# ziyu0425/PDE-Solver

Hardware: NVIDIA B200
Metric: GDOF/s (higher is better)
Workload: dtype f64

## Files before the change

### include/pde_b200.h

```cpp
#ifndef PDE_B200_H
#define PDE_B200_H

#include <stdint.h>

#ifdef __cplusplus
extern "C" {
#endif

typedef struct pde_ctx pde_ctx;

const char* pde_last_error(void);
int pde_version(void);
int pde_device_count(int32_t* count);
int pde_ctx_create(int device, pde_ctx** out);
int pde_ctx_destroy(pde_ctx* ctx);
int64_t pde_ctx_launch_count(pde_ctx* ctx);
int pde_ctx_sync(pde_ctx* ctx);
int pde_timer_start(pde_ctx* ctx);
int pde_timer_stop(pde_ctx* ctx, double* elapsed_ms);

int pde_host_alloc(uint64_t bytes, void** out);
int pde_host_free(void* p);

int pde_nccl_unique_id(const char* libnccl_path, void* id128 );
// ... 72 lines not shown
  pde_bc bc;
} pde_heat_params;

int pde_heat_solve(pde_ctx* ctx, const pde_heat_params* p, const pde_solver_opts* o,
                   const double* u0, double* values_out, double* times_out, pde_stats* st);

typedef struct pde_heat_state pde_heat_state;
int pde_heat_open(pde_ctx* ctx, const pde_heat_params* p, const pde_solver_opts* o,
                  pde_heat_state** out);
int pde_heat_set_state(pde_heat_state* s, const double* u_host );
int pde_heat_step(pde_heat_state* s, int nsteps, pde_stats* st);
int pde_heat_get_state(pde_heat_state* s, double* u_host );
int pde_heat_advance_batch(pde_heat_state* s, int nreq, const double* const* u_in_host,
                           double* const* u_out_host, pde_stats* st);
int64_t pde_heat_local_nverts(pde_heat_state* s);
int pde_heat_close(pde_heat_state* s);

typedef struct pde_wheat_params {
  int32_t dim;
  int32_t n[3];
  double lo[3], hi[3];
  int32_t weight_rpow;
  int32_t weight_sin_axis1;
  int32_t weight_degree;
  int32_t steady;
  double diffusivity;
  double dt;
  int32_t num_steps;
  int32_t snapshot_stride;
  double source_value;
  double T_initial;
  pde_bc bc;
  int32_t weight_kind;
  int32_t has_core;
  double core_radius;
  double core_diffusivity;
  int32_t initial_type;
  int32_t reserved0;
  double initial_amplitude;
  double initial_wavenumber;
} pde_wheat_params;
int pde_wheat_solve(pde_ctx* ctx, const pde_wheat_params* p, const pde_solver_opts* o,
                    double* values_out , double* times_out, pde_stats* st);
typedef struct pde_wheat_state pde_wheat_state;
int pde_wheat_open(pde_ctx* ctx, const pde_wheat_params* p, const pde_solver_opts* o, pde_wheat_state** out);
int pde_wheat_set_state(pde_wheat_state* s, const double* u_host );
int pde_wheat_step(pde_wheat_state* s, int nsteps, pde_stats* st);
int pde_wheat_get_state(pde_wheat_state* s, double* u_host );
int64_t pde_wheat_local_nverts(pde_wheat_state* s);
int pde_wheat_close(pde_wheat_state* s);
int pde_wheat_level_coefs(pde_ctx* ctx, const pde_wheat_params* p, int level, int32_t n_out[3], double* coef_out);

typedef struct pde_elast_params {
  int32_t dim;
  int32_t n[3];
  double L[3];
  double E;
  double nu;
  double body[3];
  int32_t quantity;
  int32_t plane_stress;
  double area;
} pde_elast_params;

int pde_elasticity_solve(pde_ctx* ctx, const pde_elast_params* p, const pde_solver_opts* o,
                         double* field_out, double* disp_out, pde_stats* st, pde_stats* st_proj);

enum { PDE_OP_HEAT = 0, PDE_OP_MASS = 1, PDE_OP_STIFFNESS = 2, PDE_OP_ELASTICITY = 3 };

typedef struct pde_op_params {
  int32_t kind;
  int32_t dim;
  int32_t n[3];
  double L[3];
  double alpha;
  double beta;
  double lam, mu;
  pde_bc bc;
  int32_t variant;
} pde_op_params;

int pde_op_table(const pde_op_params* p, double* table, int32_t* ncomp);
int pde_op_apply(pde_ctx* ctx, const pde_op_params* p, const double* x, double* y);
int pde_op_bench(pde_ctx* ctx, const pde_op_params* p, int reps, int warmup, double* ms_per_apply,
                 int64_t* ndofs);
int pde_op_sweep(pde_ctx* ctx, const pde_op_params* p, int32_t mode, double c1, double c2, const double* x,
                 const double* b, const double* xprev, double* y, double* dots);
int pde_op_bench_mode(pde_ctx* ctx, const pde_op_params* p, int32_t mode, int32_t reps, int32_t warmup,
                      double* ms_per_launch, int64_t* ndofs);
int pde_op_solve(pde_ctx* ctx, const pde_op_params* p, const pde_solver_opts* o, const double* b,
                 double* x, pde_stats* st);

int pde_op_manufactured(pde_ctx* ctx, const pde_op_params* p, const pde_solver_opts* o, double* rel_l2_error,
                        pde_stats* st);

#ifdef __cplusplus
}
#endif
#endif
```

### pde_solver_b200/_lib.py

```python
import ctypes as C
import os
import threading

import numpy as np

_HERE = os.path.dirname(os.path.abspath(__file__))
LIB_PATH = os.environ.get("PDE_B200_LIB") or os.path.join(_HERE, "libpde_b200.so")


class PdeError(RuntimeError):
    pass


class Bc(C.Structure):
    _fields_ = [("face_on", C.c_int32 * 6), ("face_val", C.c_double * 6), ("side_excludes_xends", C.c_int32)]


class SolverOpts(C.Structure):
    _fields_ = [("rtol", C.c_double), ("max_iters", C.c_int32), ("precond", C.c_int32),
                ("cheby_degree", C.c_int32), ("check_every", C.c_int32), ("cheby_ratio", C.c_double),
                ("verify_residual", C.c_int32), ("reserved", C.c_int32 * 3)]


class Stats(C.Structure):
# ... 148 lines not shown
        return ms.value

    def close(self):
        if self.handle:
            lib().pde_ctx_destroy(self.handle)
            self.handle = C.c_void_p()


_ctx = None


def default_context():
    global _ctx
    if _ctx is None:
        _ctx = Context()
    return _ctx


def device_count():
    n = C.c_int32(0)
    check(lib().pde_device_count(C.byref(n)))
    return int(n.value)


def nccl_library_path():
    try:
        import nvidia.nccl as _n
        base = list(_n.__path__)[0]
        p = os.path.join(base, "lib", "libnccl.so.2")
        if os.path.exists(p):
            return p
    except Exception:
        pass
    return None


def nccl_unique_id(libnccl_path=None):
    buf = (C.c_char * 128)()
    path = libnccl_path.encode() if libnccl_path else None
    check(lib().pde_nccl_unique_id(path, buf))
    return bytes(buf)


def mesh_counts(dim, n):
    nv, nc = C.c_int64(), C.c_int64()
    check(lib().pde_mesh_counts(int(dim), i3(n), C.byref(nv), C.byref(nc)))
    return nv.value, nc.value


def slab_partition(dim, n, rank, world, level=0):
    z0, nzl, nzg = C.c_int32(), C.c_int32(), C.c_int32()
    check(lib().pde_slab_partition(int(dim), i3(n), int(rank), int(world), int(level), C.byref(z0), C.byref(nzl),
                                   C.byref(nzg)))
    return z0.value, nzl.value, nzg.value


def op_params(kind, dim, n, L, alpha=1.0, beta=1.0, lam=0.0, mu=0.0, bc=None, variant=0):
    p = OpParams()
    p.kind = OP[kind] if isinstance(kind, str) else int(kind)
    p.dim = int(dim)
    p.n = i3(n)
    p.L = d3(L)
    p.alpha, p.beta, p.lam, p.mu = float(alpha), float(beta), float(lam), float(mu)
    p.bc = bc if bc is not None else Bc()
    p.variant = int(variant)
    return p


def op_table(p):
    nc = C.c_int32()
    check(lib().pde_op_table(C.byref(p), None, C.byref(nc)))
    t = np.zeros((27, 15, nc.value, nc.value))
    check(lib().pde_op_table(C.byref(p), ptr(t), C.byref(nc)))
    return t


def op_apply(ctx, p, x):
    x = np.ascontiguousarray(x, dtype=np.float64)
    y = np.empty_like(x)
    check(lib().pde_op_apply(ctx.handle, C.byref(p), ptr(x), ptr(y)))
    return y


def op_sweep(ctx, p, mode, x, b=None, xprev=None, c1=0.0, c2=0.0):
    x = np.ascontiguousarray(x, dtype=np.float64)
    b = None if b is None else np.ascontiguousarray(b, dtype=np.float64)
    xprev = None if xprev is None else np.ascontiguousarray(xprev, dtype=np.float64)
    y = np.empty_like(x)
    dots = np.zeros(2)
    check(lib().pde_op_sweep(ctx.handle, C.byref(p), int(mode), C.c_double(c1), C.c_double(c2), ptr(x),
                             ptr(b) if b is not None else None, ptr(xprev) if xprev is not None else None, ptr(y),
                             ptr(dots)))
    return y, dots


def op_bench_mode(ctx, p, mode, reps=20, warmup=3):
    ms, nd = C.c_double(), C.c_int64()
    check(lib().pde_op_bench_mode(ctx.handle, C.byref(p), int(mode), int(reps), int(warmup), C.byref(ms), C.byref(nd)))
    return ms.value, nd.value


def op_solve(ctx, p, b, opts=None):
    b = np.ascontiguousarray(b, dtype=np.float64)
    x = np.empty_like(b)
    st = Stats()
    o = opts if opts is not None else make_opts()
    check(lib().pde_op_solve(ctx.handle, C.byref(p), C.byref(o), ptr(b), ptr(x), C.byref(st)))
    return x, st.as_dict()


def comm_info(ctx):
    hp, ne, na = C.c_int32(), C.c_int64(), C.c_int64()
    check(lib().pde_comm_info(ctx.handle, C.byref(hp), C.byref(ne), C.byref(na)))
    return {"halo_path": {0: "none", 1: "nccl send/recv", 2: "peer-memory mailbox kernel (cudaIpc over NVLink)"}[hp.value],
            "halo_exchanges": ne.value, "allreduces": na.value}


def halo_check(ctx, dim, n, ncomp=1, depth=1, reps=4):
    bad = C.c_int64(0)
    check(lib().pde_halo_check(ctx.handle, int(dim), i3(n), int(ncomp), int(depth), int(reps), C.byref(bad)))
    return int(bad.value)


def halo_bench(ctx, dim, n, ncomp=1, reps=50):
    ms, nb = C.c_double(), C.c_int64()
    check(lib().pde_halo_bench(ctx.handle, int(dim), i3(n), int(ncomp), int(reps), C.byref(ms), C.byref(nb)))
    return ms.value, nb.value


def op_manufactured(ctx, p, opts=None):
    err = C.c_double()
    st = Stats()
    o = opts if opts is not None else make_opts()
    check(lib().pde_op_manufactured(ctx.handle, C.byref(p), C.byref(o), C.byref(err), C.byref(st)))
    return err.value, st.as_dict()


def op_bench(ctx, p, reps=20, warmup=3):
    ms, nd = C.c_double(), C.c_int64()
    check(lib().pde_op_bench(ctx.handle, C.byref(p), int(reps), int(warmup), C.byref(ms), C.byref(nd)))
    return ms.value, nd.value


class PinnedArray:

    def __init__(self, n):
        self.ptr = C.c_void_p()
        check(lib().pde_host_alloc(C.c_uint64(int(n) * 8), C.byref(self.ptr)))
        self.array = np.ctypeslib.as_array(C.cast(self.ptr, C.POINTER(C.c_double)), shape=(int(n),))

    def free(self):
        if self.ptr:
            self.array = None
            lib().pde_host_free(self.ptr)
            self.ptr = C.c_void_p()


class HeatStepper:

    def __init__(self, ctx, dim, n, L, diffusivity, dt, T_initial=0.0, bc=None, source_value=0.0, steady=False,
                 opts=None):
        p = HeatParams()
        p.dim = int(dim)
        p.n = i3(n)
        p.L = d3(L)
        p.diffusivity = float(diffusivity)
# ... 41 lines not shown
```

### pde_solver_b200/csrc/cabi.cu

```cuda
#include <cmath>
#include <cstdlib>
#include <cstring>
#include <new>

#include "solver.cuh"

int comm_destroy(pde_ctx* c);

extern "C" int pde_ctx_create(int device, pde_ctx** out) {
  if (!out) PDE_FAIL("null out pointer");
  int ndev = 0;
  cudaError_t e = cudaGetDeviceCount(&ndev);
  if (e != cudaSuccess || ndev == 0)
    PDE_FAIL(std::string("no CUDA device available (this library has no CPU fallback): ") + cudaGetErrorString(e));
  if (device < 0 || device >= ndev) PDE_FAIL("device index out of range");
  CUDA_OK(cudaSetDevice(device));
  pde_ctx* c = new (std::nothrow) pde_ctx();
  if (!c) PDE_FAIL("out of host memory");
  c->device = device;
  cudaDeviceGetAttribute(&c->sm_count, cudaDevAttrMultiProcessorCount, device);
  CUDA_OK(cudaStreamCreateWithFlags(&c->stream, cudaStreamNonBlocking));
  CUDA_OK(cudaEventCreate(&c->ev0));
  CUDA_OK(cudaEventCreate(&c->ev1));
  CUDA_OK(cudaEventCreateWithFlags(&c->ev_poll, cudaEventDisableTiming));
// ... 551 lines not shown
    if ((rc = pipe_init(s, false))) break;
    s->pipe.nout = 0;
    if ((rc = pipe_push_snapshot(s, values_out))) break;
    times_out[snap++] = 0.0;
    const int stride = p->snapshot_stride > 0 ? p->snapshot_stride : 1;
    const int verify = s->o.verify_residual;
    for (int step = 0; step < p->num_steps; ++step) {
      pde_stats st;
      s->o.verify_residual = step == p->num_steps - 1 ? verify : -1;
      if ((rc = pde_heat_step(s, 1, &st))) break;
      acc.true_relres = st.true_relres;
      acc.iters_total += st.iters_total;
      acc.solves += st.solves;
      acc.converged &= st.converged;
      acc.levels = st.levels;
      acc.final_relres = st.final_relres;
      acc.solve_ms += st.solve_ms;
      acc.launches += st.launches;
      if ((step + 1) % stride == 0) {
        if ((rc = pipe_push_snapshot(s, values_out + snap * s->nloc))) break;
        times_out[snap++] = (step + 1) * p->dt;
      }
    }
    if (!rc) rc = pipe_drain(s);
    acc.setup_ms = s->setup_ms;
  } while (0);
  pde_heat_close(s);
  if (st_out) *st_out = acc;
  return rc;
}

static int setup_op(pde_ctx* c, const pde_op_params* p, Operator* A, int* ncomp) {
  Grid g;
  PDE_OK(make_grid(p->dim, p->n, p->L, c->rank, c->world, &g));
  BcDev bc;
  PDE_OK(make_bc(p->dim, p->n, &p->bc, &bc));
  if (p->kind == PDE_OP_ELASTICITY) {
    if (p->dim < 2) PDE_FAIL("elasticity operator needs dim 2 or 3");
    PDE_OK(A->setup_elasticity(c, g, bc, p->lam, p->mu));
  } else {
    double a = p->kind == PDE_OP_MASS ? 1.0 : (p->kind == PDE_OP_STIFFNESS ? 0.0 : p->alpha);
    double b = p->kind == PDE_OP_MASS ? 0.0 : (p->kind == PDE_OP_STIFFNESS ? 1.0 : p->beta);
    PDE_OK(A->setup_scalar(c, g, bc, a, b));
  }
  *ncomp = A->tab.ncomp;
  return 0;
}

struct OpGuard {
  Operator A;
  Field x, y, r;
  PcgWork w;
  Hierarchy mg;
  ~OpGuard() { A.release(); x.release(); y.release(); r.release(); w.release(); mg.release(); }
};

extern "C" int pde_device_count(int32_t* count) {
  int n = 0;
  if (cudaGetDeviceCount(&n) != cudaSuccess) { cudaGetLastError(); n = 0; }
  if (count) *count = n;
  return 0;
}

extern "C" int pde_op_apply(pde_ctx* c, const pde_op_params* p, const double* x, double* y) {
  if (!c || !p || !x || !y) PDE_FAIL("null argument");
  CUDA_OK(cudaSetDevice(c->device));
  OpGuard G;
  int nc;
  PDE_OK(setup_op(c, p, &G.A, &nc));
  const Grid& g = G.A.g;
  PDE_OK(G.x.alloc(c, g, nc));
  PDE_OK(G.y.alloc(c, g, nc));
  const long long nloc = (long long)g.nn[0] * g.nn[1] * g.nzl;
  DevMem dense;
  PDE_OK(dense.alloc(sizeof(double) * nloc * nc));
  PDE_OK(h2d(c, dense.p, x, sizeof(double) * nloc * nc));
  PDE_OK(launch_unpack(c, g, nc, (const double*)dense.p, G.x.p, 0));
  StencilArgs a;
  a.x = G.x.p; a.y = G.y.p; a.variant = p->variant; a.reduce_slot_xy = S_XY;
  if (c->world > 1) PDE_OK(comm_halo_exchange(c, g, nc, G.x.p));
  PDE_OK(launch_stencil(c, g, G.A.bc, G.A.dev, a));
  PDE_OK(launch_pack(c, g, nc, G.y.p, (double*)dense.p, 0));
  return d2h(c, y, dense.p, sizeof(double) * nloc * nc);
}

extern "C" int pde_op_bench(pde_ctx* c, const pde_op_params* p, int reps, int warmup, double* ms_per_apply,
                            int64_t* ndofs) {
  if (!c || !p) PDE_FAIL("null argument");
  CUDA_OK(cudaSetDevice(c->device));
  OpGuard G;
  int nc;
  PDE_OK(setup_op(c, p, &G.A, &nc));
  const Grid& g = G.A.g;
  PDE_OK(G.x.alloc(c, g, nc));
  PDE_OK(G.y.alloc(c, g, nc));
  PDE_OK(launch_fill_pattern(c, g, G.A.bc, nc, G.x.p));
  StencilArgs a;
  a.x = G.x.p; a.y = G.y.p; a.variant = p->variant; a.reduce_slot_xy = S_XY;
  for (int i = 0; i < warmup; ++i) PDE_OK(launch_stencil(c, g, G.A.bc, G.A.dev, a));
  CUDA_OK(cudaEventRecord(c->ev0, c->stream));
  for (int i = 0; i < reps; ++i) PDE_OK(launch_stencil(c, g, G.A.bc, G.A.dev, a));
  CUDA_OK(cudaEventRecord(c->ev1, c->stream));
  CUDA_OK(cudaEventSynchronize(c->ev1));
  float ms = 0;
  CUDA_OK(cudaEventElapsedTime(&ms, c->ev0, c->ev1));
  if (ms_per_apply) *ms_per_apply = ms / (reps > 0 ? reps : 1);
  if (ndofs) *ndofs = (int64_t)g.nn[0] * g.nn[1] * g.nzl * nc;
  return 0;
}

static int sweep_args(int mode, double c1, double c2, const Field& x, const Field& b, Field& y, StencilArgs* a) {
  if (mode < 0 || mode > 5) PDE_FAIL("sweep mode must be 0..5");
  if (mode == 5) {
    a->x = b.p; a->y = y.p; a->cheby = 2; a->s0 = c2; a->c1 = c1; a->c2 = c2;
    return 0;
  }
  a->x = x.p; a->y = y.p;
  if (mode >= 1) a->b = b.p;
  if (mode == 1) { a->bscale = 1.0; a->ascale = -1.0; }
  if (mode >= 2) { a->cheby = 1; a->c1 = mode == 2 ? 0.0 : c1; a->c2 = c2; }
  if (mode == 3) { a->prev_mode = 1; a->xprev = y.p; }
  if (mode == 4) a->prev_mode = 2;
  return 0;
}

extern "C" int pde_op_sweep(pde_ctx* c, const pde_op_params* p, int mode, double c1, double c2, const double* x,
                            const double* b, const double* xprev, double* y, double* dots) {
  if (!c || !p || !x || !y) PDE_FAIL("null argument");
  if (mode >= 1 && !b) PDE_FAIL("this sweep mode needs b");
  if (mode == 3 && !xprev) PDE_FAIL("sweep mode 3 needs xprev");
  CUDA_OK(cudaSetDevice(c->device));
  OpGuard G;
  Field fb;
  struct Rel { Field* f; ~Rel() { f->release(); } } rel{&fb};
  int nc;
  PDE_OK(setup_op(c, p, &G.A, &nc));
  const Grid& g = G.A.g;
  PDE_OK(G.x.alloc(c, g, nc));
  PDE_OK(G.y.alloc(c, g, nc));
  PDE_OK(fb.alloc(c, g, nc));
  const long long nloc = (long long)g.nn[0] * g.nn[1] * g.nzl;
  DevMem dense;
  PDE_OK(dense.alloc(sizeof(double) * nloc * nc));
  auto up = [&](const double* h, double* padded) -> int {
    PDE_OK(h2d(c, dense.p, h, sizeof(double) * nloc * nc));
    return launch_unpack(c, g, nc, (const double*)dense.p, padded, 0);
  };
  PDE_OK(up(x, G.x.p));
  if (mode >= 1) PDE_OK(up(b, fb.p));
  if (mode == 3) PDE_OK(up(xprev, G.y.p));
  StencilArgs a;
  PDE_OK(sweep_args(mode, c1, c2, G.x, fb, G.y, &a));
  a.variant = p->variant;
  a.reduce_slot_xy = mode == 5 ? -1 : S_XY;
  CUDA_OK(cudaMemsetAsync(c->scal + S_XY, 0, 2 * sizeof(double), c->stream));
  if (c->world > 1) PDE_OK(comm_halo_exchange(c, g, nc, mode == 5 ? fb.p : G.x.p));
  PDE_OK(launch_stencil(c, g, G.A.bc, G.A.dev, a));
  if (dots) PDE_OK(read_scal(c, S_XY, 2, dots));
  PDE_OK(launch_pack(c, g, nc, G.y.p, (double*)dense.p, 0));
  return d2h(c, y, dense.p, sizeof(double) * nloc * nc);
}

extern "C" int pde_op_bench_mode(pde_ctx* c, const pde_op_params* p, int mode, int reps, int warmup, double* ms_per_launch,
                                 int64_t* ndofs) {
  if (!c || !p) PDE_FAIL("null argument");
  CUDA_OK(cudaSetDevice(c->device));
// ... 270 lines not shown
```

### pde_solver_b200/csrc/heat2.cu

```cuda
#include <cuda.h>

#include <cmath>

#include "device.cuh"
#include "tma.cuh"

namespace {

#ifndef H_RR_STAGES
#define H_RR_STAGES 3
#endif
template <bool RR>
struct HS { static constexpr int N = RR ? H_RR_STAGES : 4; };

template <int CW, int YSB>
struct HG {
  static constexpr int TX = CW - 2, YSA = YSB + 1, TY = 2 * YSB, RA = TY + 2;
  static constexpr int BX = TX + 4, BYX = TY + 4, BYB = TY + 2;
  static constexpr int XBOX = BX * BYX, BBOX = BX * BYB;
  static constexpr int XS = (XBOX + 15) / 16 * 16, BS = (BBOX + 15) / 16 * 16;
  static constexpr int STAGE = XS + BS;
  static constexpr int RING = RA * CW;
  static constexpr int NT = 2 * CW;
  static constexpr size_t smem(int nst) { return ((size_t)nst * STAGE + 4 * RING) * sizeof(double) + nst * sizeof(uint64_t); }
};

struct H2Coef {
  double c0, cxp, cxm, cyp, cym, czp, czm, cxyp, cxym, cxzp, cxzm, cyzp, cyzm, cdp, cdm;
};
struct H2Args {
  double* y;
  double a0, a1, k1;
  int do_reduce;
  double* yc;
  int cnn0, cnn1, cnzl, cz0, cPX;
  long long cplane;
};
struct H2Geom {
  int nn0, nn1, nzl, z0, nzg, PX;
  long long plane;
  int ntx, nty, nzc, zc;
};

template <int YS>
__device__ __forceinline__ void h2_contrib(const H2Coef& C, const double (&V)[YS + 2][3], double (&aP)[YS], double (&a0)[YS],
                                           double (&aM)[YS]) {
#pragma unroll
  for (int j = 0; j < YS; ++j) {
    const int r = j + 1;
    double t = fma(C.c0, V[r][1], a0[j]);
    t = fma(C.cxp, V[r][2], t);
    t = fma(C.cxm, V[r][0], t);
    t = fma(C.cyp, V[r + 1][1], t);
    t = fma(C.cym, V[r - 1][1], t);
    t = fma(C.cxyp, V[r + 1][2], t);
    a0[j] = fma(C.cxym, V[r - 1][0], t);
    double p = fma(C.czp, V[r][1], aP[j]);
    p = fma(C.cxzp, V[r][2], p);
    p = fma(C.cyzp, V[r + 1][1], p);
    aP[j] = fma(C.cdp, V[r + 1][2], p);
    double m = C.czm * V[r][1];
    m = fma(C.cxzm, V[r][0], m);
    m = fma(C.cyzm, V[r - 1][1], m);
    aM[j] = fma(C.cdm, V[r - 1][0], m);
  }
}

template <int CW, int YSB, bool RR>
__global__ void __launch_bounds__(2 * CW, CW == 64 ? ((RR && H_RR_STAGES == 3) ? 4 : (YSB >= 4 ? 3 : (YSB == 3 ? 4 : 5))) : 6)
k_heat_post2(const __grid_constant__ CUtensorMap tmx, const __grid_constant__ CUtensorMap tmb,
             const __grid_constant__ H2Coef C, const __grid_constant__ H2Args a, const __grid_constant__ H2Geom ge,
             ReduceBuf red, double* red_out) {
  using G = HG<CW, YSB>;
  constexpr int YSA = G::YSA;
  constexpr int H_STAGES = HS<RR>::N;
  extern __shared__ __align__(128) unsigned char smem_raw[];
  double* const stage0 = reinterpret_cast<double*>(smem_raw);
  double* const ring0 = stage0 + H_STAGES * G::STAGE;
  uint64_t* const bars = reinterpret_cast<uint64_t*>(ring0 + 4 * G::RING);

  const int t = threadIdx.x;
  const int item = blockIdx.x;
  const int itx = item % ge.ntx;
  const int ity = (item / ge.ntx) % ge.nty;
  const int izc = item / (ge.ntx * ge.nty);
  const int x0 = itx * G::TX, y0 = ity * G::TY;
  const int za = izc * ge.zc;
  const int zb = min(za + ge.zc, ge.nzl);
  const int nplanes = zb - za + 4;
  const uint32_t bar0 = smem_u32(bars);
  const uint32_t stg0 = smem_u32(stage0);
  constexpr uint32_t STAGE_BYTES = G::STAGE * 8;

  auto issue = [&](int n) {
    const uint32_t bar = bar0 + 8 * (n % H_STAGES);
    const uint32_t dst = stg0 + (n % H_STAGES) * STAGE_BYTES;
    mbar_expect_tx(bar, (uint32_t)((G::XBOX + (n >= 2 ? G::BBOX : 0)) * 8));
    tma_load_4d(dst, &tmx, x0 - 2, y0 - 2, za - 2 + n + PDE_NG, 0, bar);
    if (n >= 2) tma_load_4d(dst + G::XS * 8, &tmb, x0 - 2, y0 - 1, za - 3 + n + PDE_NG, 0, bar);
  };
  if (t == 0) {
#pragma unroll
    for (int s = 0; s < H_STAGES; ++s) mbar_init(bar0 + 8 * s, 1);
    asm volatile("fence.mbarrier_init.release.cluster;" ::: "memory");
  }
  __syncthreads();
  if (t == 0)
    for (int n = 0; n < 2 && n < nplanes; ++n) issue(n);

  const int c = t % CW;
  const int s = t / CW;
  const int ix = x0 - 1 + c;
  const int cB = min(max(c, 1), CW - 2);
  const bool xfree = ix >= 1 && ix <= ge.nn0 - 2;
  unsigned mAb = 0, mBb = 0, okB = 0;
#pragma unroll
  for (int j = 0; j < YSA; ++j) {
    const int iy = y0 - 1 + s * YSA + j;
    if (xfree && iy >= 1 && iy <= ge.nn1 - 2) mAb |= 1u << j;
  }
#pragma unroll
  for (int j = 0; j < YSB; ++j) {
    const int iy = y0 + s * YSB + j;
    const bool in = c >= 1 && c <= G::TX && ix < ge.nn0 && iy < ge.nn1;
    if (in) okB |= 1u << j;
    if (in && xfree && iy >= 1 && iy <= ge.nn1 - 2) mBb |= 1u << j;
  }
  const int offA = (s * YSA) * G::BX + c;
  const int offbA = G::XS + (s * YSA) * G::BX + c + 1;
  const int offbB = G::XS + (s * YSB + 1) * G::BX + cB + 1;
  const int offxB = (s * YSB + 2) * G::BX + cB + 1;
  const int ringA = (s * YSA) * CW + c;
  const int ringB = (s * YSB) * CW + cB - 1;
  double* yrun = a.y + ((long long)ge.PX * (y0 + s * YSB) + ix) + ge.plane * za;

  double aA[YSA], aB[YSA], aC[YSA];
  double bA_[YSB], bB_[YSB], bC_[YSB];
#pragma unroll
  for (int j = 0; j < YSA; ++j) aA[j] = aB[j] = aC[j] = 0.0;
#pragma unroll
  for (int j = 0; j < YSB; ++j) bA_[j] = bB_[j] = bC_[j] = 0.0;
  double red_by = 0.0;

  auto body = [&](int i, double (&aP)[YSA], double (&a0)[YSA], double (&aM)[YSA], double (&bP)[YSB], double (&b0)[YSB],
                  double (&bM)[YSB]) {
    const int stage = i % H_STAGES;
    const int q = za - 2 + i;
    const int pA = q - 1;
    const int pB = q - 2;
    const bool finA = i >= 2, finB = i >= 4;
    double xB0[YSB], bvB[YSB];
    if (!RR && finB) {
      const double* const sx2 = stage0 + ((i - 2) % H_STAGES) * G::STAGE + offxB;
      const double* const sb1 = stage0 + ((i - 1) % H_STAGES) * G::STAGE + offbB;
#pragma unroll
      for (int j = 0; j < YSB; ++j) { xB0[j] = sx2[j * G::BX]; bvB[j] = sb1[j * G::BX]; }
    }
    mbar_wait(bar0 + 8 * stage, (uint32_t)((i / H_STAGES) & 1));
    const double* const sx = stage0 + stage * G::STAGE;
    {
      double V[YSA + 2][3];
      const double* const sp = sx + offA;
#pragma unroll
      for (int r = 0; r < YSA + 2; ++r)
#pragma unroll
        for (int cc = 0; cc < 3; ++cc)
          V[r][cc] = ((r == 0 && cc == 2) || (r == YSA + 1 && cc == 0)) ? 0.0 : sp[r * G::BX + cc];
      h2_contrib<YSA>(C, V, aP, a0, aM);
    }
    if (finA) {
      const int gz = pA + ge.z0;
      const bool zfree = gz >= 1 && gz <= ge.nzg - 2;
      const unsigned mA = zfree ? mAb : 0u;
      double* const ds = ring0 + ((pA + 4) & 3) * G::RING + ringA;
      const double* const sb = sx + offbA;
#pragma unroll
      for (int j = 0; j < YSA; ++j) ds[j * CW] = ((mA >> j) & 1u) ? a.a0 * (sb[j * G::BX] - aP[j]) : 0.0;
    }
    __syncthreads();
    if (t == 0 && i + 2 < nplanes) issue(i + 2);
    if (!RR && finA) {
      double V[YSB + 2][3];
      const double* const rp = ring0 + ((pA + 4) & 3) * G::RING + ringB;
#pragma unroll
      for (int r = 0; r < YSB + 2; ++r)
#pragma unroll
        for (int cc = 0; cc < 3; ++cc)
          V[r][cc] = ((r == 0 && cc == 2) || (r == YSB + 1 && cc == 0)) ? 0.0 : rp[r * CW + cc];
      h2_contrib<YSB>(C, V, bP, b0, bM);
    }
    if (RR && finB) {
      const int gz = pB + ge.z0;
      const int Z = (gz >> 1) - a.cz0;
      constexpr int NCX = G::TX / 2, NCY = G::TY / 2;
      if (!(gz & 1) && Z >= 0 && Z < a.cnzl && t < NCX * NCY) {
        const int cx = t % NCX, cy = t / NCX;
        const int X = (x0 >> 1) + cx, Y = (y0 >> 1) + cy;
        if (X < a.cnn0 && Y < a.cnn1) {
          const int o = (1 + 2 * cy) * CW + 1 + 2 * cx;
          const double* const r0 = ring0 + ((pB + 4) & 3) * G::RING + o;
          const double* const rm = ring0 + ((pB + 3) & 3) * G::RING + o;
          const double* const rp = ring0 + ((pB + 5) & 3) * G::RING + o;
          const double nb = ((r0[1] + r0[-1]) + (r0[CW] + r0[-CW])) + ((r0[CW + 1] + r0[-CW - 1]) + (rp[0] + rm[0])) +
                            ((rp[1] + rm[-1]) + (rp[CW] + rm[-CW])) + (rp[CW + 1] + rm[-CW - 1]);
          const int cgz = gz >> 1;
          const bool cfree = X >= 1 && X <= a.cnn0 - 2 && Y >= 1 && Y <= a.cnn1 - 2 && cgz >= 1 && cgz <= (ge.nzg >> 1) - 1;
          a.yc[(long long)a.cPX * Y + a.cplane * Z + X] = cfree ? fma(0.5, nb, r0[0]) : 0.0;
        }
      }
    }
    if (!RR && finB) {
      const int gz = pB + ge.z0;
      const bool zfree = gz >= 1 && gz <= ge.nzg - 2;
      const unsigned mB = zfree ? mBb : 0u;
      const double* const dso = ring0 + ((pB + 4) & 3) * G::RING + ringB + CW + 1;
#pragma unroll
      for (int j = 0; j < YSB; ++j) {
        const bool m = (mB >> j) & 1u;
        const double x2 = m ? fma(a.k1, dso[j * CW], fma(-a.a1, bP[j], xB0[j])) : xB0[j];
        if ((okB >> j) & 1u) yrun[j * (long long)ge.PX] = x2;
        red_by = fma(m ? bvB[j] : 0.0, x2, red_by);
      }
      yrun += ge.plane;
    }
  };

  for (int i = 0; i < nplanes; i += 3) {
    body(i, aA, aB, aC, bB_, bC_, bA_);
    if (i + 1 < nplanes) body(i + 1, aB, aC, aA, bC_, bA_, bB_);
    if (i + 2 < nplanes) body(i + 2, aC, aA, aB, bA_, bB_, bC_);
  }
  if (a.do_reduce) {
    double v[1] = {red_by};
    block_reduce_finalize<1>(v, red, red_out);
  }
}

template <int CW, int YSB, bool RR>
int launch_t(pde_ctx* c, const Grid& g, const OpDev& op, const double* x0, const double* b, const H2Args& ha_in) {
  using G = HG<CW, YSB>;
  H2Geom ge;
  ge.nn0 = g.nn[0]; ge.nn1 = g.nn[1]; ge.nzl = g.nzl; ge.z0 = g.z0; ge.nzg = g.nzg; ge.PX = g.PX; ge.plane = g.plane;
  ge.ntx = (g.nn[0] + G::TX - 1) / G::TX;
  ge.nty = (g.nn[1] + G::TY - 1) / G::TY;
  static const int zc_env = env_int("PDE_B200_P2_ZC", 64);
  int zc = zc_env < 4 ? 4 : zc_env;
  while (zc > 8 && (long long)ge.ntx * ge.nty * ((g.nzl + zc - 1) / zc) < 6LL * c->sm_count) zc /= 2;
  ge.nzc = (g.nzl + zc - 1) / zc;
  ge.zc = (g.nzl + ge.nzc - 1) / ge.nzc;
  ge.nzc = (g.nzl + ge.zc - 1) / ge.zc;
  const long long items = (long long)ge.ntx * ge.nty * ge.nzc;
  if (items > RED_MAX_BLOCKS) return 2;
  auto kern = k_heat_post2<CW, YSB, RR>;
  static bool attr_set = false;
  if (!attr_set) {
    CUDA_OK(cudaFuncSetAttribute(kern, cudaFuncAttributeMaxDynamicSharedMemorySize, (int)G::smem(HS<RR>::N)));
    CUDA_OK(cudaFuncSetAttribute(kern, cudaFuncAttributePreferredSharedMemoryCarveout, 100));
    attr_set = true;
  }
  CUtensorMap tmx, tmb;
  PDE_OK(field_tensor_map(x0, g, 1, G::BX, G::BYX, &tmx));
  PDE_OK(field_tensor_map(b, g, 1, G::BX, G::BYB, &tmb));
  H2Coef C;
  const double* h = op.h_int;
  C.c0 = h[0]; C.cxp = h[1]; C.cxm = h[2]; C.cyp = h[3]; C.cym = h[4]; C.czp = h[5]; C.czm = h[6]; C.cxyp = h[7];
  C.cxym = h[8]; C.cxzp = h[9]; C.cxzm = h[10]; C.cyzp = h[11]; C.cyzm = h[12]; C.cdp = h[13]; C.cdm = h[14];
  kern<<<(unsigned)items, G::NT, G::smem(HS<RR>::N), c->stream>>>(tmx, tmb, C, ha_in, ge, c->red, ha_in.do_reduce ? c->scal + ha_in.do_reduce - 1 : nullptr);
  c->launches++;
  CUDA_OK(cudaGetLastError());
  return 0;
}

bool heat2_applicable(const Grid& g, const OpDev& op) {
  static const int off = env_int("PDE_B200_NO_HEAT2", 0);
  if (off) return false;
  if (g.dim != 3 || g.nk != PDE_NOFF || op.ncomp != 1 || !op.uniform_diag) return false;
  return g.nn[0] >= 32 && g.nn[1] >= 8 && g.nzl >= 8;
}

template <bool RR>
int dispatch(pde_ctx* c, const Grid& g, const OpDev& op, const double* x0, const double* b, const H2Args& ha) {
  static const int cw_env = env_int("PDE_B200_P2_CW", 0);
  static const int ysb = env_int("PDE_B200_P2_YSB", 4);
  const int cw = cw_env ? cw_env : (g.nn[0] >= 128 ? 64 : 32);
  if (cw == 64 && ysb == 3) return launch_t<64, 3, RR>(c, g, op, x0, b, ha);
  if (cw == 64) return launch_t<64, 4, RR>(c, g, op, x0, b, ha);
  return launch_t<32, 4, RR>(c, g, op, x0, b, ha);
}

}

bool post2_applicable(const Grid& g, const OpDev& op) {
  if (g.dim != 3 || g.nk != PDE_NOFF || op.ncomp != 1 || !op.uniform_diag) return false;
  if (g.nn[0] < 32 || g.nn[1] < 8 || g.nzl < 8) return false;
  return !env_int("PDE_B200_NO_HEAT2", 0) || !env_int("PDE_B200_NO_POST2", 0);
}

int launch_heat_post2(pde_ctx* c, const Grid& g, const OpDev& op, const double* x0, const double* b, double* y, double c2_0,
                      double c1_1, double c2_1, int dot_slot, bool* handled) {
  *handled = false;
  if (!heat2_applicable(g, op) || !(c2_0 * op.h_dinv_int[0] > 0.0)) return 0;
  H2Args ha{};
  ha.y = y;
  ha.a0 = c2_0 * op.h_dinv_int[0];
  ha.a1 = c2_1 * op.h_dinv_int[0];
  ha.k1 = 1.0 + c1_1 + ha.a1 / ha.a0;
  ha.do_reduce = dot_slot >= 0 ? dot_slot + 1 : 0;
  const int rc = dispatch<false>(c, g, op, x0, b, ha);
  if (rc == 0) *handled = true;
  return rc == 2 ? 0 : rc;
}

int launch_heat_resid_restrict(pde_ctx* c, const Grid& gf, const Grid& gc, const OpDev& op, const double* x, const double* b,
                               double* bcoarse, bool* handled) {
  *handled = false;
  static const int off = env_int("PDE_B200_NO_RR", 0);
  if (off || !heat2_applicable(gf, op)) return 0;
  if (gf.nc[0] != 2 * gc.nc[0] || gf.nc[1] != 2 * gc.nc[1] || gf.nc[2] != 2 * gc.nc[2] || gf.z0 != 2 * gc.z0) return 0;
  H2Args ha{};
  ha.a0 = 1.0;
  ha.yc = bcoarse;
  ha.cnn0 = gc.nn[0]; ha.cnn1 = gc.nn[1]; ha.cnzl = gc.nzl; ha.cz0 = gc.z0; ha.cPX = gc.PX; ha.cplane = gc.plane;
  const int rc = dispatch<true>(c, gf, op, x, b, ha);
  if (rc == 0) *handled = true;
  return rc == 2 ? 0 : rc;
}
```

### pde_solver_b200/csrc/kernels.cu

```cuda
#include <cstring>

#include "device.cuh"
#include "tma.cuh"

template <int NC>
struct IntCoef {
  double c[PDE_NOFF][NC * NC];
};

struct StencilDev {
  const double* x;
  const double* b;
  double* y;
  const double* xprev;
  int prev_mode;
  double bconst[3];
  double bscale, ascale, c1, c2, s0;
  int do_reduce;
  int first2;
  double* defer;
};

template <int NC, bool CHEBY>
__global__ void __launch_bounds__(128)
// ... 875 lines not shown

template <int NC>
__global__ void __launch_bounds__(256)
k_restrict(const __grid_constant__ Grid gf, const __grid_constant__ Grid gc, const __grid_constant__ BcDev bcc,
           const double* __restrict__ rf, double* __restrict__ bc_out) {
  const unsigned n0 = (unsigned)gc.nn[0], n1 = (unsigned)gc.nn[1];
  const long long total = (long long)n0 * n1 * gc.nzl;
  const bool small = total < (1LL << 32);
  for (long long t = (long long)blockIdx.x * blockDim.x + threadIdx.x; t < total; t += (long long)gridDim.x * blockDim.x) {
    const unsigned row = small ? (unsigned)t / n0 : (unsigned)(t / n0);
    const int ix = (int)(t - (long long)row * n0);
    const int iy = (int)(row % n1);
    const int lz = (int)(row / n1);
    const int gz = lz + gc.z0;
    const long long cbase = (long long)gc.PX * iy + gc.plane * lz;
    const int fy = gf.nc[1] > 0 ? 2 * iy : 0;
    const int flz = (gf.nc[2] > 0 ? 2 * gz : 0) - gf.z0;
    const long long fi = (long long)gf.PX * fy + gf.plane * flz + 2 * ix;
    double bcv;
    const bool isdir = bc_node(gc, bcc, ix, iy, gz, &bcv);
#pragma unroll
    for (int i = 0; i < NC; ++i) {
      double s = 0.0;
      if (!isdir) {
        const double* rp = rf + i * gf.comp_stride;
        double nb = 0.0;
        for (int k = 1; k < gf.nk; ++k) nb += rp[fi + gf.koff[k]];
        s = rp[fi] + 0.5 * nb;
      }
      bc_out[cbase + ix + i * gc.comp_stride] = s;
    }
  }
}

int launch_restrict(pde_ctx* c, const Grid& gf, const Grid& gc, const BcDev& bcc, int ncomp, const double* rf,
                    double* bcoarse) {
  const int blocks = flat_blocks(c, (long long)gc.nn[0] * gc.nn[1] * gc.nzl, 256);
  DISPATCH_NC(ncomp, (k_restrict<NC><<<blocks, 256, 0, c->stream>>>(gf, gc, bcc, rf, bcoarse)));
  c->launches++;
  CUDA_OK(cudaGetLastError());
  return 0;
}

template <int NC>
__global__ void __launch_bounds__(256)
k_prolong_add(const __grid_constant__ Grid gf, const __grid_constant__ Grid gc, const __grid_constant__ BcDev bcf,
              const double* __restrict__ xc, double* __restrict__ xf, int ghost) {
  const int nzr = gf.nzl + 2 * ghost;
  const unsigned npair = (unsigned)(gf.nn[0] + 1) / 2;
  const long long total = (long long)gf.nn[1] * nzr * npair;
  const bool small = total < (1LL << 32);
  for (long long t = (long long)blockIdx.x * blockDim.x + threadIdx.x; t < total; t += (long long)gridDim.x * blockDim.x) {
    const unsigned row = small ? (unsigned)t / npair : (unsigned)(t / npair);
    const int k = (int)(t - (long long)row * npair);
    const int iy = (int)(row % (unsigned)gf.nn[1]);
    const int lz = (int)(row / (unsigned)gf.nn[1]) - ghost;
    const int gz = lz + gf.z0;
    if (gz < 0 || gz > gf.nzg - 1) continue;
    const int ix = 2 * k;
    double bcv;
    const bool f0 = !bc_node(gf, bcf, ix, iy, gz, &bcv);
    const bool f1 = ix + 1 < gf.nn[0] && !bc_node(gf, bcf, ix + 1, iy, gz, &bcv);
    if (!f0 && !f1) continue;
    const long long fbase = (long long)gf.PX * iy + gf.plane * lz;
    const int py = gf.nc[1] > 0 ? (iy & 1) : 0;
    const int pz = gf.nc[2] > 0 ? (gz & 1) : 0;
    const int cy = gf.nc[1] > 0 ? (iy - py) / 2 : 0;
    const int clz = (gf.nc[2] > 0 ? (gz - pz) / 2 : 0) - gc.z0;
    const long long lo = (long long)gc.PX * cy + gc.plane * clz + k;
    const long long cpy = (long long)gc.PX * py + gc.plane * pz;
#pragma unroll
    for (int i = 0; i < NC; ++i) {
      const double* cp = xc + i * gc.comp_stride;
      double2* fp = reinterpret_cast<double2*>(xf + fbase + ix + i * gf.comp_stride);
      double2 v = *fp;
      const double c0 = cp[lo];
      if (f0) v.x += 0.5 * (c0 + cp[lo + cpy]);
      if (f1) v.y += 0.5 * (c0 + cp[lo + 1 + cpy]);
      *fp = v;
    }
  }
}

int launch_prolong_add(pde_ctx* c, const Grid& gf, const Grid& gc, const BcDev& bcf, int ncomp, const double* xc,
                       double* xf, int ghost) {
  const long long total = (long long)gf.nn[1] * (gf.nzl + 2 * ghost) * ((gf.nn[0] + 1) / 2);
  if (gf.nn[1] * (long long)(gf.nzl + 2 * ghost) >= (1LL << 32)) PDE_FAIL("prolongation: too many rows");
  const int blocks = flat_blocks(c, total, 256);
  DISPATCH_NC(ncomp, (k_prolong_add<NC><<<blocks, 256, 0, c->stream>>>(gf, gc, bcf, xc, xf, ghost)));
  c->launches++;
  CUDA_OK(cudaGetLastError());
  return 0;
}

__global__ void __launch_bounds__(256)
k_dense_solve(int n, const double* __restrict__ Ainv, const long long* __restrict__ idx, const double* __restrict__ b,
              double* __restrict__ x) {
  const int warp = (blockIdx.x * blockDim.x + threadIdx.x) >> 5, lane = threadIdx.x & 31;
  if (warp >= n) return;
  double s = 0.0;
  for (int j = lane; j < n; j += 32) s = fma(Ainv[(size_t)warp * n + j], b[idx[j]], s);
#pragma unroll
  for (int o = 16; o > 0; o >>= 1) s += __shfl_down_sync(0xffffffffu, s, o);
  if (lane == 0) x[idx[warp]] = s;
}

int launch_dense_solve(pde_ctx* c, int n, const double* Ainv, const long long* idx, const double* b, double* x) {
  if (n <= 0) return 0;
  int blocks = (n * 32 + 255) / 256;
  k_dense_solve<<<blocks, 256, 0, c->stream>>>(n, Ainv, idx, b, x);
  c->launches++;
  CUDA_OK(cudaGetLastError());
  return 0;
}

__global__ void __launch_bounds__(256)
k_dense_gather(int n, const long long* __restrict__ idx, const double* __restrict__ b, double* __restrict__ bglob) {
  const int j = blockIdx.x * blockDim.x + threadIdx.x;
  if (j < n) bglob[j] = idx[j] >= 0 ? b[idx[j]] : 0.0;
}
__global__ void __launch_bounds__(256)
k_dense_solve_owned(int n, const double* __restrict__ Ainv, const long long* __restrict__ idx,
                    const double* __restrict__ bglob, double* __restrict__ x) {
  const int warp = (blockIdx.x * blockDim.x + threadIdx.x) >> 5, lane = threadIdx.x & 31;
  if (warp >= n || idx[warp] < 0) return;
  double s = 0.0;
  for (int j = lane; j < n; j += 32) s = fma(Ainv[(size_t)warp * n + j], bglob[j], s);
#pragma unroll
  for (int o = 16; o > 0; o >>= 1) s += __shfl_down_sync(0xffffffffu, s, o);
  if (lane == 0) x[idx[warp]] = s;
}
int launch_dense_gather(pde_ctx* c, int n, const long long* idx, const double* b, double* bglob) {
  if (n <= 0) return 0;
  k_dense_gather<<<(n + 255) / 256, 256, 0, c->stream>>>(n, idx, b, bglob);
  c->launches++;
  CUDA_OK(cudaGetLastError());
  return 0;
}
int launch_dense_solve_owned(pde_ctx* c, int n, const double* Ainv, const long long* idx, const double* bglob,
                             double* x) {
  if (n <= 0) return 0;
  k_dense_solve_owned<<<(n * 32 + 255) / 256, 256, 0, c->stream>>>(n, Ainv, idx, bglob, x);
  c->launches++;
  CUDA_OK(cudaGetLastError());
  return 0;
}

__global__ void __launch_bounds__(128)
k_fill_ic(const __grid_constant__ Grid g, const __grid_constant__ BcDev bc, double* __restrict__ u, double value,
          int fill, int apply_bc) {
  const long long rows = (long long)g.nn[1] * g.nzl;
  for (long long row = (long long)blockIdx.x * blockDim.y + threadIdx.y; row < rows;
       row += (long long)gridDim.x * blockDim.y) {
    const int iy = (int)(row % g.nn[1]);
    const int lz = (int)(row / g.nn[1]);
    const long long rbase = (long long)g.PX * iy + g.plane * lz;
    for (int ix = threadIdx.x; ix < g.nn[0]; ix += blockDim.x) {
      double bcv;
      const bool isdir = apply_bc && bc_node(g, bc, ix, iy, lz + g.z0, &bcv);
      if (isdir) u[rbase + ix] = bcv;
      else if (fill) u[rbase + ix] = value;
    }
  }
}
__global__ void __launch_bounds__(128)
k_fill_pattern(const __grid_constant__ Grid g, const __grid_constant__ BcDev bc, int ncomp, double* __restrict__ x) {
  const long long rows = (long long)g.nn[1] * g.nzl;
  for (long long row = (long long)blockIdx.x * blockDim.y + threadIdx.y; row < rows;
       row += (long long)gridDim.x * blockDim.y) {
    const int iy = (int)(row % g.nn[1]);
    const int lz = (int)(row / g.nn[1]);
    for (int ix = threadIdx.x; ix < g.nn[0]; ix += blockDim.x) {
// ... 550 lines not shown
```

Measured before the change: 2.674.

## Add row-wise warp prolongation kernel and carry heat2 B-stage operands in registers

Adds a warp-per-row-chunk prolongation kernel for scalar fields. It hoists boundary checks per row and batches loads for several pairs per lane to raise memory-level parallelism, replacing the per-pair thread kernel when ncomp is 1. In the heat2 fused kernel, the non-RR path now keeps the x and b values needed by the lagging B stage in small register rings captured during the A stage, instead of rereading them from older shared-memory stages. Both paths now use a fixed 3-stage pipeline. It also adds a test entry point for prolongation. The register rings raise register pressure, and the non-RR path now runs 3 stages instead of 4.

New measurement: 2.696, median of 6. Within noise of the previous version (+0.8%).

```diff
diff --git a/include/pde_b200.h b/include/pde_b200.h
--- a/include/pde_b200.h
+++ b/include/pde_b200.h
@@ -178,6 +178,7 @@
 
 int pde_op_table(const pde_op_params* p, double* table, int32_t* ncomp);
 int pde_op_apply(pde_ctx* ctx, const pde_op_params* p, const double* x, double* y);
+int pde_op_prolong_add(pde_ctx* ctx, const pde_op_params* p, const double* xc, double* xf);
 int pde_op_bench(pde_ctx* ctx, const pde_op_params* p, int reps, int warmup, double* ms_per_apply,
                  int64_t* ndofs);
 int pde_op_sweep(pde_ctx* ctx, const pde_op_params* p, int32_t mode, double c1, double c2, const double* x,
diff --git a/pde_solver_b200/_lib.py b/pde_solver_b200/_lib.py
--- a/pde_solver_b200/_lib.py
+++ b/pde_solver_b200/_lib.py
@@ -254,6 +254,13 @@
     return y
 
 
+def op_prolong_add(ctx, p, xc, xf):
+    xc = np.ascontiguousarray(xc, dtype=np.float64)
+    y = np.array(xf, dtype=np.float64, order="C")
+    check(lib().pde_op_prolong_add(ctx.handle, C.byref(p), ptr(xc), ptr(y)))
+    return y
+
+
 def op_sweep(ctx, p, mode, x, b=None, xprev=None, c1=0.0, c2=0.0):
     x = np.ascontiguousarray(x, dtype=np.float64)
     b = None if b is None else np.ascontiguousarray(b, dtype=np.float64)
diff --git a/pde_solver_b200/csrc/cabi.cu b/pde_solver_b200/csrc/cabi.cu
--- a/pde_solver_b200/csrc/cabi.cu
+++ b/pde_solver_b200/csrc/cabi.cu
@@ -657,6 +657,35 @@
   PDE_OK(launch_stencil(c, g, G.A.bc, G.A.dev, a));
   PDE_OK(launch_pack(c, g, nc, G.y.p, (double*)dense.p, 0));
   return d2h(c, y, dense.p, sizeof(double) * nloc * nc);
+}
+
+extern "C" int pde_op_prolong_add(pde_ctx* c, const pde_op_params* p, const double* xc, double* xf) {
+  if (!c || !p || !xc || !xf) PDE_FAIL("null argument");
+  if (c->world > 1) PDE_FAIL("prolongation entry: single rank only");
+  CUDA_OK(cudaSetDevice(c->device));
+  int32_t nh[3] = {p->n[0], p->n[1], p->n[2]};
+  for (int d = 0; d < p->dim; ++d) {
+    if (p->n[d] < 2 || p->n[d] % 2) PDE_FAIL("prolongation entry: cell counts must be even");
+    nh[d] = p->n[d] / 2;
+  }
+  OpGuard G;
+  int nc;
+  PDE_OK(setup_op(c, p, &G.A, &nc));
+  const Grid& g = G.A.g;
+  Grid gc;
+  PDE_OK(make_grid(p->dim, nh, p->L, 0, 1, &gc));
+  PDE_OK(G.x.alloc(c, g, nc));
+  PDE_OK(G.y.alloc(c, gc, nc));
+  const long long nf = (long long)g.nn[0] * g.nn[1] * g.nzl, ncv = (long long)gc.nn[0] * gc.nn[1] * gc.nzl;
+  DevMem dense;
+  PDE_OK(dense.alloc(sizeof(double) * nf * nc));
+  PDE_OK(h2d(c, dense.p, xc, sizeof(double) * ncv * nc));
+  PDE_OK(launch_unpack(c, gc, nc, (const double*)dense.p, G.y.p, 0));
+  PDE_OK(h2d(c, dense.p, xf, sizeof(double) * nf * nc));
+  PDE_OK(launch_unpack(c, g, nc, (const double*)dense.p, G.x.p, 0));
+  PDE_OK(launch_prolong_add(c, g, gc, G.A.bc, nc, G.y.p, G.x.p, 0));
+  PDE_OK(launch_pack(c, g, nc, G.x.p, (double*)dense.p, 0));
+  return d2h(c, xf, dense.p, sizeof(double) * nf * nc);
 }
 
 extern "C" int pde_op_bench(pde_ctx* c, const pde_op_params* p, int reps, int warmup, double* ms_per_apply,
diff --git a/pde_solver_b200/csrc/heat2.cu b/pde_solver_b200/csrc/heat2.cu
--- a/pde_solver_b200/csrc/heat2.cu
+++ b/pde_solver_b200/csrc/heat2.cu
@@ -7,11 +7,7 @@
 
 namespace {
 
-#ifndef H_RR_STAGES
-#define H_RR_STAGES 3
-#endif
-template <bool RR>
-struct HS { static constexpr int N = RR ? H_RR_STAGES : 4; };
+constexpr int H_STAGES = 3;
 
 template <int CW, int YSB>
 struct HG {
@@ -67,13 +63,12 @@
 }
 
 template <int CW, int YSB, bool RR>
-__global__ void __launch_bounds__(2 * CW, CW == 64 ? ((RR && H_RR_STAGES == 3) ? 4 : (YSB >= 4 ? 3 : (YSB == 3 ? 4 : 5))) : 6)
+__global__ void __launch_bounds__(2 * CW, CW == 64 ? (RR ? 4 : (YSB >= 4 ? 3 : (YSB == 3 ? 4 : 5))) : 6)
 k_heat_post2(const __grid_constant__ CUtensorMap tmx, const __grid_constant__ CUtensorMap tmb,
              const __grid_constant__ H2Coef C, const __grid_constant__ H2Args a, const __grid_constant__ H2Geom ge,
              ReduceBuf red, double* red_out) {
   using G = HG<CW, YSB>;
   constexpr int YSA = G::YSA;
-  constexpr int H_STAGES = HS<RR>::N;
   extern __shared__ __align__(128) unsigned char smem_raw[];
   double* const stage0 = reinterpret_cast<double*>(smem_raw);
   double* const ring0 = stage0 + H_STAGES * G::STAGE;
@@ -128,34 +123,26 @@
   }
   const int offA = (s * YSA) * G::BX + c;
   const int offbA = G::XS + (s * YSA) * G::BX + c + 1;
-  const int offbB = G::XS + (s * YSB + 1) * G::BX + cB + 1;
-  const int offxB = (s * YSB + 2) * G::BX + cB + 1;
   const int ringA = (s * YSA) * CW + c;
   const int ringB = (s * YSB) * CW + cB - 1;
   double* yrun = a.y + ((long long)ge.PX * (y0 + s * YSB) + ix) + ge.plane * za;
 
   double aA[YSA], aB[YSA], aC[YSA];
   double bA_[YSB], bB_[YSB], bC_[YSB];
+  double xo[3][YSB], bo[3][YSB];
 #pragma unroll
   for (int j = 0; j < YSA; ++j) aA[j] = aB[j] = aC[j] = 0.0;
 #pragma unroll
-  for (int j = 0; j < YSB; ++j) bA_[j] = bB_[j] = bC_[j] = 0.0;
+  for (int j = 0; j < YSB; ++j) bA_[j] = bB_[j] = bC_[j] = xo[0][j] = xo[1][j] = xo[2][j] = bo[0][j] = bo[1][j] = bo[2][j] = 0.0;
   double red_by = 0.0;
 
-  auto body = [&](int i, double (&aP)[YSA], double (&a0)[YSA], double (&aM)[YSA], double (&bP)[YSB], double (&b0)[YSB],
-                  double (&bM)[YSB]) {
+  auto body = [&](int i, int i3, double (&aP)[YSA], double (&a0)[YSA], double (&aM)[YSA], double (&bP)[YSB],
+                  double (&b0)[YSB], double (&bM)[YSB]) {
     const int stage = i % H_STAGES;
     const int q = za - 2 + i;
     const int pA = q - 1;
     const int pB = q - 2;
     const bool finA = i >= 2, finB = i >= 4;
-    double xB0[YSB], bvB[YSB];
-    if (!RR && finB) {
-      const double* const sx2 = stage0 + ((i - 2) % H_STAGES) * G::STAGE + offxB;
-      const double* const sb1 = stage0 + ((i - 1) % H_STAGES) * G::STAGE + offbB;
-#pragma unroll
-      for (int j = 0; j < YSB; ++j) { xB0[j] = sx2[j * G::BX]; bvB[j] = sb1[j * G::BX]; }
-    }
     mbar_wait(bar0 + 8 * stage, (uint32_t)((i / H_STAGES) & 1));
     const double* const sx = stage0 + stage * G::STAGE;
     {
@@ -167,6 +154,10 @@
         for (int cc = 0; cc < 3; ++cc)
           V[r][cc] = ((r == 0 && cc == 2) || (r == YSA + 1 && cc == 0)) ? 0.0 : sp[r * G::BX + cc];
       h2_contrib<YSA>(C, V, aP, a0, aM);
+      if (!RR) {
+#pragma unroll
+        for (int j = 0; j < YSB; ++j) xo[i3][j] = s ? V[j + 1][1] : V[j + 2][1];
+      }
     }
     if (finA) {
       const int gz = pA + ge.z0;
@@ -174,8 +165,16 @@
       const unsigned mA = zfree ? mAb : 0u;
       double* const ds = ring0 + ((pA + 4) & 3) * G::RING + ringA;
       const double* const sb = sx + offbA;
-#pragma unroll
-      for (int j = 0; j < YSA; ++j) ds[j * CW] = ((mA >> j) & 1u) ? a.a0 * (sb[j * G::BX] - aP[j]) : 0.0;
+      double bv[YSA];
+#pragma unroll
+      for (int j = 0; j < YSA; ++j) {
+        bv[j] = sb[j * G::BX];
+        ds[j * CW] = ((mA >> j) & 1u) ? a.a0 * (bv[j] - aP[j]) : 0.0;
+      }
+      if (!RR) {
+#pragma unroll
+        for (int j = 0; j < YSB; ++j) bo[i3][j] = s ? bv[j] : bv[j + 1];
+      }
     }
     __syncthreads();
     if (t == 0 && i + 2 < nplanes) issue(i + 2);
@@ -217,18 +216,19 @@
 #pragma unroll
       for (int j = 0; j < YSB; ++j) {
         const bool m = (mB >> j) & 1u;
-        const double x2 = m ? fma(a.k1, dso[j * CW], fma(-a.a1, bP[j], xB0[j])) : xB0[j];
+        const double xB0 = xo[(i3 + 1) % 3][j], bvB = bo[(i3 + 2) % 3][j];
+        const double x2 = m ? fma(a.k1, dso[j * CW], fma(-a.a1, bP[j], xB0)) : xB0;
         if ((okB >> j) & 1u) yrun[j * (long long)ge.PX] = x2;
-        red_by = fma(m ? bvB[j] : 0.0, x2, red_by);
+        red_by = fma(m ? bvB : 0.0, x2, red_by);
       }
       yrun += ge.plane;
     }
   };
 
   for (int i = 0; i < nplanes; i += 3) {
-    body(i, aA, aB, aC, bB_, bC_, bA_);
-    if (i + 1 < nplanes) body(i + 1, aB, aC, aA, bC_, bA_, bB_);
-    if (i + 2 < nplanes) body(i + 2, aC, aA, aB, bA_, bB_, bC_);
+    body(i, 0, aA, aB, aC, bB_, bC_, bA_);
+    if (i + 1 < nplanes) body(i + 1, 1, aB, aC, aA, bC_, bA_, bB_);
+    if (i + 2 < nplanes) body(i + 2, 2, aC, aA, aB, bA_, bB_, bC_);
   }
   if (a.do_reduce) {
     double v[1] = {red_by};
@@ -254,7 +254,7 @@
   auto kern = k_heat_post2<CW, YSB, RR>;
   static bool attr_set = false;
   if (!attr_set) {
-    CUDA_OK(cudaFuncSetAttribute(kern, cudaFuncAttributeMaxDynamicSharedMemorySize, (int)G::smem(HS<RR>::N)));
+    CUDA_OK(cudaFuncSetAttribute(kern, cudaFuncAttributeMaxDynamicSharedMemorySize, (int)G::smem(H_STAGES)));
     CUDA_OK(cudaFuncSetAttribute(kern, cudaFuncAttributePreferredSharedMemoryCarveout, 100));
     attr_set = true;
   }
@@ -265,7 +265,7 @@
   const double* h = op.h_int;
   C.c0 = h[0]; C.cxp = h[1]; C.cxm = h[2]; C.cyp = h[3]; C.cym = h[4]; C.czp = h[5]; C.czm = h[6]; C.cxyp = h[7];
   C.cxym = h[8]; C.cxzp = h[9]; C.cxzm = h[10]; C.cyzp = h[11]; C.cyzm = h[12]; C.cdp = h[13]; C.cdm = h[14];
-  kern<<<(unsigned)items, G::NT, G::smem(HS<RR>::N), c->stream>>>(tmx, tmb, C, ha_in, ge, c->red, ha_in.do_reduce ? c->scal + ha_in.do_reduce - 1 : nullptr);
+  kern<<<(unsigned)items, G::NT, G::smem(H_STAGES), c->stream>>>(tmx, tmb, C, ha_in, ge, c->red, ha_in.do_reduce ? c->scal + ha_in.do_reduce - 1 : nullptr);
   c->launches++;
   CUDA_OK(cudaGetLastError());
   return 0;
diff --git a/pde_solver_b200/csrc/kernels.cu b/pde_solver_b200/csrc/kernels.cu
--- a/pde_solver_b200/csrc/kernels.cu
+++ b/pde_solver_b200/csrc/kernels.cu
@@ -981,12 +981,95 @@
   }
 }
 
+constexpr int PROLONG_PPL = 4;
+
+__global__ void __launch_bounds__(256, 4)
+k_prolong_add_rows(const __grid_constant__ Grid gf, const __grid_constant__ Grid gc, const __grid_constant__ BcDev bcf,
+                   const double* __restrict__ xc, double* __restrict__ xf, int ghost, int nchunk, int clen) {
+  constexpr int PPL = PROLONG_PPL, NC = 1;
+  const int nzr = gf.nzl + 2 * ghost;
+  const int npair = (gf.nn[0] + 1) / 2;
+  const long long units = (long long)gf.nn[1] * nzr * nchunk;
+  const int lane = threadIdx.x & 31;
+  const long long wstride = (long long)gridDim.x * (blockDim.x >> 5);
+  for (long long u = (long long)blockIdx.x * (blockDim.x >> 5) + (threadIdx.x >> 5); u < units; u += wstride) {
+    const unsigned row = (unsigned)(u / nchunk);
+    const int ch = (int)(u - (long long)row * nchunk);
+    const int iy = (int)(row % (unsigned)gf.nn[1]);
+    const int lz = (int)(row / (unsigned)gf.nn[1]) - ghost;
+    const int gz = lz + gf.z0;
+    if (gz < 0 || gz > gf.nzg - 1) continue;
+    const bool rowdir = (gf.nc[1] > 0 && ((iy == 0 && bcf.on[2]) || (iy == gf.nn[1] - 1 && bcf.on[3]))) ||
+                        (gf.nc[2] > 0 && ((gz == 0 && bcf.on[4]) || (gz == gf.nzg - 1 && bcf.on[5])));
+    double bcv;
+    const bool free_first = !bc_node(gf, bcf, 0, iy, gz, &bcv), free_last = !bc_node(gf, bcf, gf.nn[0] - 1, iy, gz, &bcv);
+    auto is_free = [&](int ix) {
+      return ix == 0 ? free_first : (ix == gf.nn[0] - 1 ? free_last : (ix < gf.nn[0] && !rowdir));
+    };
+    const long long fbase = (long long)gf.PX * iy + gf.plane * lz;
+    const int py = gf.nc[1] > 0 ? (iy & 1) : 0;
+    const int pz = gf.nc[2] > 0 ? (gz & 1) : 0;
+    const int cy = gf.nc[1] > 0 ? (iy - py) / 2 : 0;
+    const int clz = (gf.nc[2] > 0 ? (gz - pz) / 2 : 0) - gc.z0;
+    const long long lo = (long long)gc.PX * cy + gc.plane * clz;
+    const long long cpy = (long long)gc.PX * py + gc.plane * pz;
+    const int kb = ch * clen, ke = min(kb + clen, npair);
+    bool f0[PPL], f1[PPL];
+    double2 v[PPL][NC];
+    double c0[PPL][NC], c1[PPL][NC], c2[PPL][NC];
+#pragma unroll
+    for (int j = 0; j < PPL; ++j) {
+      const int k = kb + 32 * j + lane;
+      const bool act = k < ke;
+      f0[j] = act && is_free(2 * k);
+      f1[j] = act && is_free(2 * k + 1);
+#pragma unroll
+      for (int i = 0; i < NC; ++i) {
+        const double* cp = xc + i * gc.comp_stride + lo + k;
+        if (f0[j] || f1[j]) {
+          v[j][i] = *reinterpret_cast<const double2*>(xf + fbase + 2 * k + i * gf.comp_stride);
+          c0[j][i] = cp[0];
+        }
+        if (f0[j]) c1[j][i] = cp[cpy];
+        if (f1[j]) c2[j][i] = cp[1 + cpy];
+      }
+    }
+#pragma unroll
+    for (int j = 0; j < PPL; ++j) {
+      if (!f0[j] && !f1[j]) continue;
+      const int k = kb + 32 * j + lane;
+#pragma unroll
+      for (int i = 0; i < NC; ++i) {
+        double2 w = v[j][i];
+        if (f0[j]) w.x += 0.5 * (c0[j][i] + c1[j][i]);
+        if (f1[j]) w.y += 0.5 * (c0[j][i] + c2[j][i]);
+        *reinterpret_cast<double2*>(xf + fbase + 2 * k + i * gf.comp_stride) = w;
+      }
+    }
+  }
+}
+
+static void prolong_add_rows(pde_ctx* c, const Grid& gf, const Grid& gc, const BcDev& bcf, const double* xc, double* xf,
+                             int ghost) {
+  constexpr int CMAX = 32 * PROLONG_PPL;
+  const int npair = (gf.nn[0] + 1) / 2;
+  const int nchunk = (npair + CMAX - 1) / CMAX;
+  const int clen = (npair + nchunk - 1) / nchunk;
+  const long long warps = (long long)gf.nn[1] * (gf.nzl + 2 * ghost) * nchunk;
+  const int blocks = flat_blocks(c, warps * 32, 256);
+  k_prolong_add_rows<<<blocks, 256, 0, c->stream>>>(gf, gc, bcf, xc, xf, ghost, nchunk, clen);
+}
+
 int launch_prolong_add(pde_ctx* c, const Grid& gf, const Grid& gc, const BcDev& bcf, int ncomp, const double* xc,
                        double* xf, int ghost) {
-  const long long total = (long long)gf.nn[1] * (gf.nzl + 2 * ghost) * ((gf.nn[0] + 1) / 2);
   if (gf.nn[1] * (long long)(gf.nzl + 2 * ghost) >= (1LL << 32)) PDE_FAIL("prolongation: too many rows");
-  const int blocks = flat_blocks(c, total, 256);
-  DISPATCH_NC(ncomp, (k_prolong_add<NC><<<blocks, 256, 0, c->stream>>>(gf, gc, bcf, xc, xf, ghost)));
+  if (ncomp == 1) {
+    prolong_add_rows(c, gf, gc, bcf, xc, xf, ghost);
+  } else {
+    const long long total = (long long)gf.nn[1] * (gf.nzl + 2 * ghost) * ((gf.nn[0] + 1) / 2);
+    const int blocks = flat_blocks(c, total, 256);
+    DISPATCH_NC(ncomp, (k_prolong_add<NC><<<blocks, 256, 0, c->stream>>>(gf, gc, bcf, xc, xf, ghost)));
+  }
   c->launches++;
   CUDA_OK(cudaGetLastError());
   return 0;
```
